# JiGuang283/Ray_Tracing-Rendering

Measured on AMD Instinct MI355X. Metric: Msamples/sec, Cornell Box 800x800 spp=400 MIS, higher is better.
Workload: dtype f64

## Files before the change

include/rtr_hip.h:

```cpp
#ifndef RTR_HIP_H
#define RTR_HIP_H

#include <stdint.h>
#include <stddef.h>

#ifdef __cplusplus
extern "C" {
#endif

#define RTR_ABI_VERSION 4

typedef enum rtr_status {
    RTR_OK = 0,
    RTR_ERR_INVALID = -1,
    RTR_ERR_UNSUPPORTED = -2,
    RTR_ERR_DEVICE = -3,
    RTR_ERR_NO_SCENE = -4,
    RTR_ERR_CANCELLED = -5,
    RTR_ERR_NOMEM = -6
} rtr_status;


typedef enum rtr_node_type {
    RTR_NODE_BVH = 0,
// ... 137 lines not shown
    int32_t max_depth;
    int32_t rr_start_depth;
    int32_t integrator;
    uint32_t seed;
    int32_t pipeline;
    int32_t tile_first;
    int32_t tile_stride;
    int32_t spp_chunks;
    int32_t flags;
} rtr_render_params;

#define RTR_FLAG_REFERENCE_ORDER 1
#define RTR_FLAG_WF_PERSISTENT 2
#define RTR_FLAG_SORTED_SHADING 4
#define RTR_FLAG_SPLIT_CASTS 8

typedef struct rtr_render_stats {
    uint64_t samples;
    uint64_t closest_segments;
    uint64_t shadow_segments;
    double device_ms;
    int32_t kernel_launches;
    int32_t pipeline;
    int32_t spp_chunks;
    int32_t cancelled;
    int32_t flags_in_effect;
    int32_t reserved;
} rtr_render_stats;

typedef struct rtr_context rtr_context;
// ... 198 lines not shown
```

ray_tracing-rendering_amd/_abi.py:

```python
import ctypes as C

import numpy as np

RTR_ABI_VERSION = 4

RTR_OK = 0
RTR_ERR_INVALID = -1
RTR_ERR_UNSUPPORTED = -2
RTR_ERR_DEVICE = -3
RTR_ERR_NO_SCENE = -4
RTR_ERR_CANCELLED = -5
RTR_ERR_NOMEM = -6

(NODE_BVH, NODE_LIST, NODE_TRANSLATE, NODE_ROTATE_Y, NODE_FLIP_FACE, NODE_MEDIUM, NODE_SPHERE,
 NODE_MOVING_SPHERE, NODE_XY_RECT, NODE_XZ_RECT, NODE_YZ_RECT) = range(11)
MAT_LAMBERTIAN, MAT_METAL, MAT_DIELECTRIC, MAT_DIFFUSE_LIGHT, MAT_PBR, MAT_ISOTROPIC = range(6)
TEX_SOLID, TEX_CHECKER, TEX_NOISE, TEX_IMAGE = range(4)
LIGHT_QUAD, LIGHT_POINT, LIGHT_SPOT, LIGHT_DIRECTIONAL, LIGHT_ENV_UNIFORM, LIGHT_ENV_MAP = 0, 1, 2, 3, 4, 5

INTEGRATOR_PATH, INTEGRATOR_RR, INTEGRATOR_PBR, INTEGRATOR_NEE, INTEGRATOR_MIS = 0, 1, 2, 3, 4
PIPELINE_AUTO, PIPELINE_MEGAKERNEL, PIPELINE_WAVEFRONT = 0, 1, 2
FLAG_REFERENCE_ORDER = 1
FLAG_WF_PERSISTENT = 2
FLAG_SORTED_SHADING = 4
FLAG_SPLIT_CASTS = 8
ACCUM_MOMENTS = 1

NODE_DTYPE = np.dtype([("type", "<i4"), ("a", "<i4"), ("b", "<i4"), ("reserved", "<i4"), ("f", "<f8", (10,))])
MATERIAL_DTYPE = np.dtype([("type", "<i4"), ("tex", "<i4", (4,)), ("reserved", "<i4", (3,)), ("f", "<f8", (4,))])
TEXTURE_DTYPE = np.dtype([("type", "<i4"), ("a", "<i4"), ("b", "<i4"), ("reserved", "<i4"), ("f", "<f8", (4,))])
PERLIN_DTYPE = np.dtype([("ranvec", "<f8", (256, 3)), ("perm_x", "<i4", (256,)), ("perm_y", "<i4", (256,)),
                         ("perm_z", "<i4", (256,))])
IMAGE_DTYPE = np.dtype([("width", "<i4"), ("height", "<i4"), ("offset", "<u8")])
LIGHT_DTYPE = np.dtype([("type", "<i4"), ("reserved", "<i4"), ("f", "<f8", (16,))])
CAMERA_DTYPE = np.dtype([("origin", "<f8", (3,)), ("lower_left_corner", "<f8", (3,)), ("horizontal", "<f8", (3,)),
                         ("vertical", "<f8", (3,)), ("u", "<f8", (3,)), ("v", "<f8", (3,)), ("w", "<f8", (3,)),
                         ("lens_radius", "<f8"), ("time0", "<f8"), ("time1", "<f8")])
assert NODE_DTYPE.itemsize == 96 and MATERIAL_DTYPE.itemsize == 64 and TEXTURE_DTYPE.itemsize == 48
assert PERLIN_DTYPE.itemsize == 9216 and IMAGE_DTYPE.itemsize == 16 and LIGHT_DTYPE.itemsize == 136
assert CAMERA_DTYPE.itemsize == 192
# ... 131 lines not shown
```

ray_tracing-rendering_amd/csrc/rt_kernels.h:

```cpp
#pragma once

#include "rt_render.h"

#ifndef RTR_MEGA_WAVES
#define RTR_MEGA_WAVES 4
#endif
#ifndef RTR_PROGRAM_WAVES
#define RTR_PROGRAM_WAVES 3
#endif

constexpr int mega_waves(int integ, int trav, int ms) {
    if (ms == RT_MS_LEAN) return RTR_MEGA_WAVES;
    if (rt_is_program(trav)) return RTR_PROGRAM_WAVES;
    if (trav == RT_TRAV_MEDIA || trav == RT_TRAV_EXACT) return 2;
    if (ms == RT_MS_QUADLIT) return 3;
    if (integ == RTR_INTEGRATOR_RR || integ == RTR_INTEGRATOR_PATH) return 3;
    return 2;
}

#define RT_PARK_WORDS 19
struct Park {
    double* base;
    RT_DEV V3 get3(int k) const { return mk(base[k * RTR_BLOCK], base[(k + 1) * RTR_BLOCK], base[(k + 2) * RTR_BLOCK]); }
    RT_DEV void set3(int k, V3 v) const {
// ... 521 lines not shown
    if (ACC == 2) P.q_part[(size_t)cell * RTR_BLOCK + threadIdx.x] = q;
    unsigned long long a = wave_sum(n_samples), b = wave_sum(cnt.closest), c = wave_sum(cnt.shadow);
    if ((threadIdx.x & 63) == 0) {
        atomicAdd(&P.stats[0], a);
        atomicAdd(&P.stats[1], b);
        atomicAdd(&P.stats[2], c);
    }
    const int interrupted = __syncthreads_or(active && s < s_end);
    if (threadIdx.x == 0) {
        P.done[cell] = !interrupted;
        if (interrupted) atomicAdd(&P.stats[7], 1ull);
    }
}


struct LiOut {
    double L[3];
    uint32_t rng_exit;
    int32_t n_closest, n_shadow, pad;
};
template <int INTEG, int TRAV>
__global__ void __launch_bounds__(RTR_BLOCK) k_li(const DScene sc, const RenderK P, const int32_t* __restrict__ ijs,
                                                   const rtr_li_ray* __restrict__ rays, LiOut* __restrict__ out, long long n) {
    extern __shared__ int lds_stack[];
    const Stack st{lds_stack + threadIdx.x};
    const long long k = (long long)blockIdx.x * RTR_BLOCK + threadIdx.x;
    if (k >= n) return;
    uint32_t rng;
    V3 ro, rd;
    Real tm;
// ... 145 lines not shown
    const bool cast = !rtr_ray_bad(r, media != 0);
    if (__any(cast && !(r.t_min >= 0x1p-100))) sc.shared_div = 0;
    if (cast) {
        blocked = cast_shadow<TRAV>(sc, ld3(r.origin), ld3(r.direction), r.t_max, rng, st, r.time, r.t_min);
    }
    occluded[k] = blocked ? 1 : 0;
    if (rng_out) rng_out[k] = rng;
}

#ifdef RTR_TU_CAPI
__global__ void __launch_bounds__(RTR_BLOCK) k_resolve(const ResolveK R) {
    const RenderK& P = R.r;
    int i, j;
    bool active;
    tile_pixel(P, blockIdx.x, threadIdx.x, i, j, active);
    for (int c = 0; c < P.chunks; ++c)
        if (!P.done[blockIdx.x * P.chunks + c]) return;
    const bool packed = R.row_stride < 0;
    if (packed && threadIdx.x == 0) R.tile_done[blockIdx.x] = 1;
    if (!active) return;
    const double* in = P.partial + (size_t)blockIdx.x * P.chunks * 3 * RTR_BLOCK + threadIdx.x;
    double r = 0, g = 0, b = 0;
    for (int c = 0; c < P.chunks; ++c) {
        if (c == 0) {
            r = in[0], g = in[RTR_BLOCK], b = in[2 * RTR_BLOCK];
        } else {
            r += in[0], g += in[RTR_BLOCK], b += in[2 * RTR_BLOCK];
        }
        in += 3 * RTR_BLOCK;
    }
    const double scale = 1.0 / P.spp;
    double* o = packed ? R.out + ((long long)blockIdx.x * RTR_BLOCK + threadIdx.x) * 3
// ... 615 lines not shown
```

ray_tracing-rendering_amd/csrc/rt_launch.h:

```cpp
#pragma once

#include "rt_render.h"

#include <atomic>
#include <string>
#include <utility>

struct LaunchedKernel {
    int trav = -1;
    int ms = -1;
    int sorted = 0;
    int phases = 0;
};

struct MegaVariant {
    int integ, trav, ms;
    bool sorted, pair;
};

struct MegaLaunch {
    MegaVariant variant;
    int accum;
    size_t lds;
    int stack_words;
    hipStream_t stream;
    const DScene* dsc;
    RenderK P;
    bool dry;
    int* blocks_per_cu;
};
int rtr_mega_launch_mis(const MegaLaunch& L, std::string& err);
int rtr_mega_launch_rr_path(const MegaLaunch& L, std::string& err);
int rtr_mega_launch_pbr_nee(const MegaLaunch& L, std::string& err);

void rtr_launch_resolve(const ResolveK& R, hipStream_t stream);

template <typename K>
int kernel_lds(K kernel, size_t dynamic_bytes, size_t static_bytes, std::string& err) {
    if (dynamic_bytes + static_bytes > 160 * 1024) {
        err = "this traversal of the scene needs a deeper stack than 160 KiB of LDS holds";
        return RTR_ERR_UNSUPPORTED;
    }
    if (dynamic_bytes <= 64 * 1024) return RTR_OK;
    const hipError_t e = hipFuncSetAttribute(reinterpret_cast<const void*>(kernel), hipFuncAttributeMaxDynamicSharedMemorySize,
// ... 32 lines not shown
```

ray_tracing-rendering_amd/csrc/rt_render.h:

```cpp
#pragma once

#include "rt_device.h"

struct RenderK {
    int W, H;
    int x0, y0, x1, y1;
    int spp, max_depth, rr_start;
    uint32_t seed;
    int tiles_x, tiles_y;
    const int* tile_ids;
    int n_tiles;
    int chunks;
    int n_big, big_spp, small_spp;
    int integrator;
    double* partial;
    unsigned long long* stats;
    const uint32_t* cancel;
    uint32_t render_id;
    int* done;
    const int* tile_s0;
    const double* acc_in;
    const int* tile_s1;
    const int* active;
    const int* n_active;
// ... 11 lines not shown
    const int tile = P.tile_ids[slot];
    const int tile_y = (P.tiles_y - 1) - tile / P.tiles_x;
    const int tile_x = tile % P.tiles_x;
    i = tile_x * 16 + (tid & 15);
    j = tile_y * 16 + (tid >> 4);
    active = i >= P.x0 && i < P.x1 && j >= P.y0 && j < P.y1;
}

RT_DEV void camera_sample(const DScene& sc, const RenderK& P, int i, int j, int s, uint32_t& rng, V3& ro, V3& rd, Real& tm) {
    rng = rtr_sample_seed_inline(P.seed, P.W, i, j, s);
    const Real u = (i + rng_next(rng)) / (P.W - 1);
    const Real v = (j + rng_next(rng)) / (P.H - 1);
    camera_get_ray(sc.camera, u, v, rng, ro, rd, tm);
}

RT_DEV void chunk_range(const RenderK& P, int c, int& s0, int& s1) {
    if (P.small_spp == 0) {
        s0 = (int)((long long)c * P.spp / P.chunks);
        s1 = (int)((long long)(c + 1) * P.spp / P.chunks);
    } else if (c < P.n_big) {
        s0 = c * P.big_spp, s1 = s0 + P.big_spp;
    } else {
        s0 = P.n_big * P.big_spp + (c - P.n_big) * P.small_spp, s1 = s0 + P.small_spp;
    }
    s0 = s0 < P.spp ? s0 : P.spp;
    s1 = s1 < P.spp ? s1 : P.spp;
    if (c == P.chunks - 1) s1 = P.spp;
}
RT_DEV void mega_work(const RenderK& P, int b, int& tile_slot, int& c) {
    if (P.small_spp == 0) {
        tile_slot = b / P.chunks, c = b % P.chunks;
    } else if (b < P.n_tiles * P.n_big) {
        tile_slot = b / P.n_big, c = b % P.n_big;
    } else {
        const int n_small = P.chunks - P.n_big, q = b - P.n_tiles * P.n_big;
        tile_slot = q / n_small, c = P.n_big + q % n_small;
    }
}

RT_DEV unsigned long long wave_sum(unsigned long long v) {
#pragma unroll
    for (int off = 32; off > 0; off >>= 1) v += __shfl_down(v, off, 64);
    return v;
}

struct ResolveK {
    RenderK r;
    double* out;
    long long row_stride;
    unsigned char* tile_done;
};

struct AccumResolveK {
    RenderK r;
    const double* sum;
    const int* count;
    double* out;
    unsigned char* rgb8;
};
```

ray_tracing-rendering_amd/csrc/rtr_capi.hip:

```cpp
#define RTR_TU_CAPI
#include "rt_lower.h"
#include "rt_kernels.h"
#include "rt_launch.h"
#include "rt_machine.h"
#include "rt_debug.h"

#include <atomic>
#include <cstdio>
#include <cstring>
#include <functional>
#include <map>
#include <mutex>
#include <string>
#include <vector>

namespace {

thread_local std::string g_create_error;

struct DevBuf {
    void* p = nullptr;
    size_t cap = 0;
};
struct SceneBufs {
// ... 372 lines not shown
int params_check(rtr_context* c, const rtr_render_params* p) {
    if (!p) return fail(c, RTR_ERR_INVALID, "null params");
    if (p->image_width < 2 || p->image_height < 2) return fail(c, RTR_ERR_INVALID, "image smaller than 2x2");
    if (((int64_t)p->image_width + 15) / 16 * (((int64_t)p->image_height + 15) / 16) > ((int64_t)1 << 26))
        return fail(c, RTR_ERR_INVALID, "image larger than 2^26 tiles");
    if (p->x0 < 0 || p->y0 < 0 || p->x1 > p->image_width || p->y1 > p->image_height || p->x0 >= p->x1 ||
        p->y0 >= p->y1)
        return fail(c, RTR_ERR_INVALID, "region outside the image or empty");
    if (p->spp < 1 || p->max_depth < 1 || p->rr_start_depth < 0)
        return fail(c, RTR_ERR_INVALID, "spp/max_depth/rr_start_depth out of range");
    if (p->integrator < RTR_INTEGRATOR_PATH || p->integrator > RTR_INTEGRATOR_MIS)
        return fail(c, RTR_ERR_UNSUPPORTED, "integrator id not supported (0 path, 1 RR, 2 PBR, 3 NEE, 4 MIS)");
    if (p->tile_stride > 1 && (p->tile_first < 0 || p->tile_first >= p->tile_stride))
        return fail(c, RTR_ERR_INVALID, "tile_first must be in [0, tile_stride)");
    if (p->spp_chunks < 0 || p->spp_chunks > p->spp) return fail(c, RTR_ERR_INVALID, "spp_chunks must be in [0, spp]");
    if (p->flags & ~(RTR_FLAG_REFERENCE_ORDER | RTR_FLAG_WF_PERSISTENT | RTR_FLAG_SORTED_SHADING | RTR_FLAG_SPLIT_CASTS)) return fail(c, RTR_ERR_INVALID, "unknown flag bits");
    if (p->pipeline < RTR_PIPELINE_AUTO || p->pipeline > RTR_PIPELINE_WAVEFRONT)
        return fail(c, RTR_ERR_INVALID, "unknown pipeline");
    return RTR_OK;
}

std::vector<int> owned_tiles(const rtr_render_params& p, int& tiles_x, int& tiles_y) {
    tiles_x = (p.image_width + 15) / 16;
    tiles_y = (p.image_height + 15) / 16;
    const int stride = p.tile_stride > 1 ? p.tile_stride : 1;
    const int first = p.tile_stride > 1 ? p.tile_first : 0;
    std::vector<int> out;
    for (int t = first; t < tiles_x * tiles_y; t += stride) {
        int ty = (tiles_y - 1) - t / tiles_x, tx = t % tiles_x;
        int xs = tx * 16, ys = ty * 16;
        if (xs + 16 <= p.x0 || xs >= p.x1 || ys + 16 <= p.y0 || ys >= p.y1) continue;
// ... 40 lines not shown
    if (v.trav == RT_TRAV_PROGRAM && (f.guarded_program || n1)) v.trav = RT_TRAV_PROGRAM_EXT;
    if (n1) {
        if (v.trav == RT_TRAV_EXACT) v.trav = RT_TRAV_MEDIA;
        return v;
    }
    const int t = v.trav;
    const bool lean = f.lean_materials && (t == RT_TRAV_FLAT || t == RT_TRAV_FAST || t == RT_TRAV_TOP || t == RT_TRAV_EXACT);
    const bool quadlit = f.quad_lights_only && !f.needs_uv && integ == RTR_INTEGRATOR_MIS && t != RT_TRAV_MEDIA && t != RT_TRAV_EXACT;
    v.ms = lean ? RT_MS_LEAN : (quadlit ? RT_MS_QUADLIT : RT_MS_FULL);
    v.sorted = (flags & RTR_FLAG_SORTED_SHADING) && f.n_materials <= 65535 && mega_sortable(integ, t, v.ms);
    const bool pairable = mega_pairable(integ, t) && !v.sorted && f.pair_cast;
    v.pair = pairable && !(flags & RTR_FLAG_SPLIT_CASTS);
    if (flags_in_effect && v.sorted) *flags_in_effect |= RTR_FLAG_SORTED_SHADING;
    if (flags_in_effect && pairable && !v.pair) *flags_in_effect |= RTR_FLAG_SPLIT_CASTS;
    return v;
}

int launch_mega(rtr_context* c, const RenderK& P, int integrator, int trav_in, bool dry, int* blocks_per_cu, int flags,
                int* flags_in_effect = nullptr, LaunchedKernel* launched = nullptr) {
    MegaLaunch L{};
    const MegaVariant& v = L.variant = mega_variant(c->facts, integrator, trav_in, flags, flags_in_effect);
    L.stack_words = (int)(stack_bytes(c->facts, c->info, v.trav) / (RTR_BLOCK * sizeof(int)));
    L.dsc = static_cast<const DScene*>(c->sb.dscene.p);
    const int park = v.sorted ? SK_WORDS : park_words(integrator, trav_in == RT_TRAV_EXACT ? RT_TRAV_EXACT : v.trav);
    L.lds = stack_bytes(c->facts, c->info, v.trav) + (size_t)park * RTR_BLOCK * sizeof(double);
    L.accum = P.tile_s0 == nullptr ? 0 : (P.q_in ? 2 : 1);
    L.stream = c->stream;
    L.P = P;
    L.dry = dry;
    L.blocks_per_cu = blocks_per_cu;
    int rc;
    switch (integrator) {
    case RTR_INTEGRATOR_MIS: rc = rtr_mega_launch_mis(L, c->err); break;
    case RTR_INTEGRATOR_RR:
    case RTR_INTEGRATOR_PATH: rc = rtr_mega_launch_rr_path(L, c->err); break;
    default: rc = rtr_mega_launch_pbr_nee(L, c->err); break;
    }
    if (rc == RTR_OK && !dry && launched) launched->trav = v.trav, launched->ms = v.ms, launched->sorted = v.sorted;
    return rc;
}

int auto_chunks(int pipeline, double resident_slots, int n_tiles, int spp) {
    int chunks = 1;
    if (pipeline == RTR_PIPELINE_WAVEFRONT) {
        while ((long long)n_tiles * chunks < 8192 && chunks * 2 * 8 <= spp && chunks < 64) chunks *= 2;
// ... 109 lines not shown
        return RTR_OK;
    }
    HIPCHK(c, hipEventSynchronize(c->ev1));
    float ms = 0;
    HIPCHK(c, hipEventElapsedTime(&ms, c->ev0, c->ev1));
    unsigned long long h[RT_STATS_WORDS] = {0};
    HIPCHK(c, hipMemcpy(h, c->b_stats.p, sizeof h, hipMemcpyDeviceToHost));
    if (getenv("RTR_REGION_PROFILE")) {
        static const char* names[RG_N] = {"other / loop", "closest: instance setup", "closest: rect runs", "closest: sphere runs",
                                          "closest: generic scan", "closest: tree inner nodes", "closest: tree leaves",
                                          "closest: hit record (fast_finish)", "shadow: instance setup", "shadow: rect runs",
                                          "shadow: sphere runs", "shadow: generic scan", "shadow: tree inner nodes",
                                          "shadow: tree leaves", "media steps", "mat_prepare", "shade_a (emission, light sample)",
                                          "shade_b (BSDF sample, roulette)", "miss", "end of sample + regeneration",
                                          "shade_rr / shade_path", "park path state", "sorted shading: barrier waits",
                                          "sorted shading: tickets + exchange", "pair cast: instance setup",
                                          "pair cast: rect runs", "pair cast: sphere runs", "sample end: cancel poll",
                                          "sample end: begin_sample (camera ray)", "sample end: settle into the pixel sum",
                                          "cast counters", "random_in_unit_sphere rejection loop"};
        double total = 0;
        for (int k = 0; k < RG_N; ++k) total += (double)h[RT_PROF_BASE + k];
        std::fprintf(stderr, "[region profile] %.4g wave cycles in all, %llu samples\n", total, h[0]);
        for (int k = 0; k < RG_N; ++k)
            if (h[RT_PROF_BASE + RT_PROF_REGIONS + k])
                std::fprintf(stderr, "[region profile] %-36s %6.2f %%  %12llu visits  %8.1f cycles/visit\n", names[k],
                             100.0 * (double)h[RT_PROF_BASE + k] / total, h[RT_PROF_BASE + RT_PROF_REGIONS + k],
                             (double)h[RT_PROF_BASE + k] / (double)h[RT_PROF_BASE + RT_PROF_REGIONS + k]);
    }
#ifdef RTR_PHASE_CLOCKS
    std::fprintf(stderr, "[phase clocks] closest %.3e  shade %.3e  shadow %.3e  other %.3e (wave cycles)\n", (double)h[3],
                 (double)h[4], (double)h[5], (double)h[6]);
// ... 219 lines not shown
    if (pipeline == RTR_PIPELINE_AUTO) pipeline = RTR_PIPELINE_MEGAKERNEL;
    const int trav = pick_trav(c->facts, c->info, p->flags);
    if (pipeline == RTR_PIPELINE_WAVEFRONT && (!c->facts.machine_ok || (trav != RT_TRAV_FLAT && trav != RT_TRAV_FAST && trav != RT_TRAV_PROGRAM)))
        return fail(c, RTR_ERR_UNSUPPORTED, "the wavefront pipeline runs the compiled traversals only: this graph (or "
                                            "RTR_FLAG_REFERENCE_ORDER) needs the reference-order walk of the megakernel");
    if (pipeline == RTR_PIPELINE_WAVEFRONT && (p->flags & RTR_FLAG_WF_PERSISTENT) && c->facts.guarded_program)
        return fail(c, RTR_ERR_UNSUPPORTED, "RTR_FLAG_WF_PERSISTENT: the traversal machine does not run step programs with "
                                            "guarded primitives (hollow spheres under bvh_nodes) or media under transforms; "
                                            "the lockstep stages do");
    int chunks = p->spp_chunks, guided[3] = {0, 0, 0};
    if (chunks == 0 && (rc = choose_chunks(c, P, p->integrator, pipeline, trav, p->spp, p->flags, &chunks, guided))) return rc;
    P.n_big = guided[0], P.big_spp = guided[1], P.small_spp = guided[2];
    P.chunks = chunks;

    const size_t partial_bytes = (size_t)P.n_tiles * chunks * 3 * RTR_BLOCK * sizeof(double);
    const size_t done_bytes = (size_t)P.n_tiles * chunks * sizeof(int);
    const bool same_tiles = acc || tiles == c->last_tiles;
    if ((c->stats_pending || c->in_flight) && (!same_tiles || partial_bytes > c->b_partial.cap || done_bytes > c->b_done.cap ||
                                               pipeline == RTR_PIPELINE_WAVEFRONT)) {
        if ((rc = finish_stats(c))) return rc;
    }
    if (!same_tiles) {
        c->last_tiles.clear();
        if ((rc = upload(c, c->b_tiles, tiles.data(), tiles.size() * sizeof(int)))) return rc;
        c->last_tiles = tiles;
    }
    if ((rc = ensure(c, c->b_partial, partial_bytes))) return rc;
    if ((rc = ensure(c, c->b_done, done_bytes))) return rc;
    P.tile_ids = static_cast<const int*>(acc ? acc->d_tiles.p : c->b_tiles.p);
    if (acc) {
        P.tile_s0 = static_cast<const int*>(acc->d_count.p);
        P.acc_in = static_cast<const double*>(acc->d_sum.p);
        P.tile_s1 = static_cast<const int*>(acc->d_s1.p);
        P.active = static_cast<const int*>(acc->d_active.p);
        P.n_active = static_cast<const int*>(acc->d_nactive.p);
        if (acc->moments) {
            P.q_in = static_cast<const double*>(acc->d_q.p);
            P.q_part = static_cast<double*>(acc->d_qpart.p);
        }
    }
    P.stats = static_cast<unsigned long long*>(c->b_stats.p);
    P.cancel = static_cast<const uint32_t*>(c->b_cancel.p);
    P.partial = static_cast<double*>(c->b_partial.p);
    P.done = static_cast<int*>(c->b_done.p);
    if (pipeline == RTR_PIPELINE_MEGAKERNEL && (rc = launch_mega(c, P, p->integrator, trav, true, nullptr, p->flags))) return rc;

    const uint32_t id = c->render_seq.fetch_add(1) + 1;
    P.render_id = id;
    c->stats_pending = false;
    c->in_flight = true;
    c->stats = rtr_render_stats{};
    c->stats.spp_chunks = chunks;
    c->last_kernel = rtr_debug_kernel{-1, -1, -1, -1, 0, 0, 0, 0, 0, 0, 0};
    LaunchedKernel launched{};
    c->pending_id = id;
    HIPCHK(c, hipMemsetAsync(c->b_stats.p, 0, RT_STATS_WORDS * sizeof(unsigned long long), c->stream));
    if (c->camera_dirty) {
        hipLaunchKernelGGL(k_camera_store, dim3(1), dim3(64), 0, c->stream, static_cast<DScene*>(c->sb.dscene.p), c->ds.camera);
        HIPCHK(c, hipGetLastError());
        c->camera_dirty = false;
// ... 27 lines not shown
            K.n_tiles = P.n_tiles;
            K.count = static_cast<const int*>(acc->d_count.p);
            K.err = static_cast<const double*>(acc->d_err.p);
            K.tile_s1 = static_cast<int*>(acc->d_s1.p);
            K.active = static_cast<int*>(acc->d_active.p);
            K.n_active = static_cast<int*>(acc->d_nactive.p);
            if (K.mode == 2) {
                hipLaunchKernelGGL(k_accum_errors, dim3((unsigned)P.n_tiles), dim3(RTR_BLOCK), 0, c->stream, accum_view(acc),
                                   static_cast<const double*>(acc->d_q.p), static_cast<double*>(acc->d_err.p));
                ++launches;
            }
            hipLaunchKernelGGL(k_accum_plan, dim3(1), dim3(1024), 0, c->stream, K);
            ++launches;
            HIPCHK(c, hipGetLastError());
        }
        if ((rc = launch_mega(c, P, p->integrator, trav, false, nullptr, p->flags, &c->stats.flags_in_effect, &launched))) return rc;
        c->last_kernel = rtr_debug_kernel{pipeline, p->integrator, launched.trav, launched.ms, launched.sorted, 0, 0, 0, 0, 0, 0,
                                          acc ? (acc->moments ? 2 : 1) : 0};
        if (acc) {
            hipLaunchKernelGGL(k_accum_commit, dim3((unsigned)P.n_tiles), dim3(RTR_BLOCK), 0, c->stream, P,
                               static_cast<double*>(acc->d_sum.p), static_cast<double*>(acc->moments ? acc->d_q.p : nullptr),
                               static_cast<int*>(acc->d_count.p));
        } else {
            ResolveK R{P, d_rgb, (long long)row_stride, tile_done};
            rtr_launch_resolve(R, c->stream);
        }
        HIPCHK(c, hipGetLastError());
        c->stats.kernel_launches = launches;
    }
    HIPCHK(c, hipEventRecord(c->ev1, c->stream));
    c->stats.pipeline = pipeline;
    c->stats_pending = true;
    if (blocking || c->stats.cancelled) {
        HIPCHK(c, hipStreamSynchronize(c->stream));
        if ((rc = finish_stats(c))) return rc;
        if (c->stats.cancelled) return fail(c, RTR_ERR_CANCELLED, "render cancelled");
    }
    return RTR_OK;
}
// ... 1193 lines not shown
```

ray_tracing-rendering_amd/csrc/rtr_mega.hip:

```cpp
#include "rt_kernels.h"
#include "rt_launch.h"

#ifndef RTR_MEGA_GROUP
#error "compile with -DRTR_MEGA_GROUP=0|1|2"
#endif

namespace {

int mega_fail(std::string& err, int code, const std::string& m) {
    err = m;
    return code;
}

template <typename K>
int launch_one(K kernel, const MegaLaunch& L, std::string& err) {
    hipFuncAttributes fa{};
    hipError_t e = hipFuncGetAttributes(&fa, reinterpret_cast<const void*>(kernel));
    if (e == hipSuccess)
        if (int rc = kernel_lds(kernel, L.lds, fa.sharedSizeBytes, err)) return rc;
    if (e == hipSuccess && L.dry && L.blocks_per_cu)
        e = hipOccupancyMaxActiveBlocksPerMultiprocessor(L.blocks_per_cu, kernel, RTR_BLOCK, L.lds);
    if (e == hipSuccess && !L.dry) {
        hipLaunchKernelGGL(kernel, dim3((unsigned)(L.P.n_tiles * L.P.chunks)), dim3(RTR_BLOCK), L.lds, L.stream, L.dsc, L.P,
                           L.stack_words);
        e = hipGetLastError();
    }
    if (e != hipSuccess) return mega_fail(err, RTR_ERR_DEVICE, std::string("megakernel launch: ") + hipGetErrorString(e));
    return RTR_OK;
}

template <int I, int T, int M, bool S = false, bool PR = false>
struct Row {
    static bool is(const MegaVariant& v) { return v.integ == I && v.trav == T && v.ms == M && v.sorted == S && v.pair == PR; }
    static int launch(const MegaLaunch& L, std::string& err) {
        return L.accum == 2 ? launch_one(k_mega<I, T, M, S, 2, PR>, L, err)
               : L.accum    ? launch_one(k_mega<I, T, M, S, 1, PR>, L, err)
                            : launch_one(k_mega<I, T, M, S, 0, PR>, L, err);
    }
};
template <typename... Rows>
int launch_from(const MegaLaunch& L, std::string& err) {
    int rc = RTR_OK;
    if (((Rows::is(L.variant) && (rc = Rows::launch(L, err), true)) || ...)) return rc;
    const MegaVariant& v = L.variant;
    return mega_fail(err, RTR_ERR_UNSUPPORTED,
                     "no megakernel instantiation for integrator " + std::to_string(v.integ) + ", traversal " + std::to_string(v.trav) +
                         ", material set " + std::to_string(v.ms) + (v.sorted ? ", sorted" : "") + (v.pair ? ", pair cast" : ""));
}

// ... 65 lines not shown
```

ray_tracing-rendering_amd/native.py:

```python
import ctypes as C
import os
import weakref

import numpy as np

from . import _abi as A
from .scene import Scene

_HERE = os.path.dirname(os.path.abspath(__file__))
_LIB = None

_STATUS = {A.RTR_ERR_INVALID: "RTR_ERR_INVALID", A.RTR_ERR_UNSUPPORTED: "RTR_ERR_UNSUPPORTED",
           A.RTR_ERR_DEVICE: "RTR_ERR_DEVICE", A.RTR_ERR_NO_SCENE: "RTR_ERR_NO_SCENE",
           A.RTR_ERR_CANCELLED: "RTR_ERR_CANCELLED", A.RTR_ERR_NOMEM: "RTR_ERR_NOMEM"}

EXPORTS = ("rtr_abi_version", "rtr_device_count", "rtr_create", "rtr_destroy", "rtr_set_stream",
           "rtr_upload_scene", "rtr_render_device", "rtr_render_host", "rtr_render_tiles_host", "rtr_plan_chunks", "rtr_li_samples", "rtr_li_rays",
           "rtr_synchronize", "rtr_cancel", "rtr_get_stats", "rtr_last_error", "rtr_sample_seed", "rtr_validate_scene",
           "rtr_accum_create", "rtr_accum_render", "rtr_accum_resolve", "rtr_accum_tiles", "rtr_accum_destroy",
           "rtr_accum_create_ex", "rtr_accum_render_tiles", "rtr_accum_moments", "rtr_accum_errors", "rtr_accum_refine",
           "rtr_denoise_defaults", "rtr_accum_features", "rtr_accum_denoise", "rtr_denoise_host",
           "rtr_query_closest", "rtr_query_occluded", "rtr_query_closest_device", "rtr_query_occluded_device",
           "rtr_set_camera", "rtr_get_camera", "rtr_accum_reset", "rtr_temporal_defaults", "rtr_history_create",
           "rtr_history_clear", "rtr_history_destroy", "rtr_history_planes", "rtr_accum_denoise_temporal",
           "rtr_display_defaults", "rtr_display_srgb_thresholds", "rtr_display_histogram", "rtr_display_host",
           "rtr_display_device", "rtr_accum_resolve_device", "rtr_accum_features_device", "rtr_accum_denoise_device",
           "rtr_accum_denoise_temporal_device")
TEST_EXPORTS = ("rtr_test_hits", "rtr_test_materials", "rtr_test_lights", "rtr_test_li", "rtr_test_reference_order",
                "rtr_test_stream8", "rtr_test_sincos_exhaustive", "rtr_test_shared_division", "rtr_test_issue_rates", "rtr_test_last_kernel",
                "rtr_test_temporal_planes", "rtr_test_scene_plan", "rtr_test_flat_hits", "rtr_test_pair_frames",
                "rtr_test_pair_frame_host", "rtr_test_pair_cast")
_TEST_LIB = None


class SceneInfoC(C.Structure):
    _fields_ = [("stack_words", C.c_int32), ("has_media", C.c_int32), ("needs_uv", C.c_int32),
                ("graph_depth", C.c_int32), ("fast_ok", C.c_int32), ("fast_instances", C.c_int32),
                ("fast_refs", C.c_int32), ("fast_stack_words", C.c_int32), ("compiled_subtrees", C.c_int32),
                ("program_steps", C.c_int32), ("inverted_boxes", C.c_int32), ("top_trees", C.c_int32)]


class KernelRecordC(C.Structure):
    _fields_ = [(name, C.c_int32) for name in ("pipeline", "integrator", "trav", "ms", "sorted", "shade_phases", "lean",
                                               "quadlit", "sort", "media", "machine", "accum")]


# ... 2 lines not shown
        "fast_ok", "has_media", "flat_scene", "flat_guarded", "lean_materials", "quad_lights_only", "uv_order_dependent",
        "machine_ok", "guarded_program", "top_tree", "needs_uv", "n_material_types", "shared_div", "pair_cast", "n_steps",
        "n_visits", "n_refs", "fast_stack_words", "walk_stack_words", "n_tie_refs", "n_guard_refs", "pick_trav", "mega_trav",
        "mega_ms", "mega_sorted", "mega_pair", "n_finish")]


FINISH_DTYPE = np.dtype([("kind", "<i4"), ("material", "<i4"), ("levels", "<i4"), ("flip", "<i4"), ("op", "<f8", (2, 3)),
                         ("g", "<f8", (4,))])


PAIR_FRAME_DTYPE = np.dtype([("ao", "<f8", (3,)), ("ad", "<f8", (3,)), ("bo", "<f8", (3,)), ("bd", "<f8", (3,)),
                             ("fo", "<f8", (3,)), ("fd", "<f8", (3,)), ("same_frame", "<i4"), ("pad", "<i4")])
PAIR_DTYPE = np.dtype([("ao", "<f8", (3,)), ("ad", "<f8", (3,)), ("a_tmax", "<f8"), ("bo", "<f8", (3,)), ("bd", "<f8", (3,)),
                       ("b_tmax", "<f8"), ("a_t", "<f8"), ("s_a_t", "<f8"), ("a_ref", "<i4"), ("a_inst", "<i4"),
                       ("b_hit", "<i4"), ("s_a_ref", "<i4"), ("s_a_inst", "<i4"), ("s_b_hit", "<i4")])
FRAME_SHAPES = ("none", "T", "R", "TR", "RT", "other")


class RtrError(RuntimeError):
    def __init__(self, code, message):
        super().__init__("%s (%d): %s" % (_STATUS.get(code, "rtr_status"), code, message))
        self.code = code
        self.message = message


def library_path():
    return os.environ.get("RTR_HIP_LIBRARY") or os.path.join(_HERE, "librtr_hip.so")


def lib():
# ... 91 lines not shown
    T.rtr_test_li.argtypes = [vp, C.POINTER(A.RenderParamsC), vp, C.c_int64]
    T.rtr_test_reference_order.argtypes = [vp, C.c_int]
    T.rtr_test_stream8.argtypes = [vp, C.c_int64, C.c_int]
    T.rtr_test_sincos_exhaustive.argtypes = [vp, C.POINTER(C.c_uint64), C.POINTER(C.c_uint64)]
    T.rtr_test_issue_rates.argtypes = [vp, C.POINTER(C.c_double), C.c_int]
    T.rtr_test_shared_division.argtypes = [vp, C.POINTER(C.c_uint64), C.POINTER(C.c_uint64)]
    T.rtr_test_last_kernel.argtypes = [vp, C.POINTER(KernelRecordC), C.c_size_t]
    T.rtr_test_temporal_planes.argtypes = [vp] + [C.c_int32] * 6 + [C.POINTER(A.CameraC), C.POINTER(A.CameraC), C.c_int,
                                                                    C.POINTER(A.TemporalParamsC)] + [vp] * 8
    T.rtr_test_scene_plan.argtypes = [C.POINTER(A.SceneDescC), C.c_int32, C.c_int32, C.POINTER(ScenePlanC), vp, C.c_int64,
                                      vp, C.c_int64]
    T.rtr_test_flat_hits.argtypes = [vp, vp, C.c_int64, C.c_int, C.POINTER(C.c_int32)]
    T.rtr_test_pair_frames.argtypes = [C.POINTER(A.SceneDescC), vp, C.c_int64, C.POINTER(C.c_int32)]
    T.rtr_test_pair_frame_host.argtypes = [C.c_int32, vp, vp, C.c_int64]
    T.rtr_test_pair_cast.argtypes = [vp, vp, C.c_int64]
    _TEST_LIB = T
    return T


def validate_scene(scene):
    L = lib()
    d = scene.desc()
    info = SceneInfoC()
    msg = C.create_string_buffer(256)
    rc = L.rtr_validate_scene(C.byref(d), C.byref(info), msg, len(msg))
    if rc != 0:
        raise RtrError(rc, msg.value.decode())
    return {"stack_words": info.stack_words, "has_media": bool(info.has_media), "needs_uv": bool(info.needs_uv),
            "graph_depth": info.graph_depth, "fast_ok": bool(info.fast_ok), "fast_instances": info.fast_instances,
            "fast_refs": info.fast_refs, "fast_stack_words": info.fast_stack_words,
# ... 26 lines not shown
    if rc != 0:
        raise RtrError(rc, "scene rejected")
    shapes = np.zeros(n.value, dtype=np.int32)
    T.rtr_test_pair_frames(C.byref(d), shapes.ctypes.data, len(shapes), C.byref(n))
    return [FRAME_SHAPES[k] for k in shapes]


def pair_frame_host(shape, ops, ao, ad, bo, bd):
    recs = np.zeros(len(ao), dtype=PAIR_FRAME_DTYPE)
    recs["ao"], recs["ad"], recs["bo"], recs["bd"] = ao, ad, bo, bd
    ops = np.ascontiguousarray(ops, dtype=np.float64).reshape(6)
    rc = test_lib().rtr_test_pair_frame_host(FRAME_SHAPES.index(shape), ops.ctypes.data, recs.ctypes.data, len(recs))
    if rc != 0:
        raise RtrError(rc, "rtr_test_pair_frame_host")
    return recs


def denoise_defaults(**overrides):
    p = A.DenoiseParamsC()
    lib().rtr_denoise_defaults(C.byref(p))
    for k, v in overrides.items():
        if k not in ("iterations", "feature_spp", "sigma_l", "sigma_n", "sigma_a", "sigma_z"):
            raise TypeError("no denoise parameter %r" % k)
        setattr(p, k, v)
    return p


def temporal_defaults(**overrides):
    p = A.TemporalParamsC()
    lib().rtr_temporal_defaults(C.byref(p))
# ... 540 lines not shown
```

Before: 5414.

## Add persistent megakernel with atomic work queue for pixel-sample jobs

Result: faster. 5734, median of 6 (+5.9%).

```diff
diff --git a/include/rtr_hip.h b/include/rtr_hip.h
--- a/include/rtr_hip.h
+++ b/include/rtr_hip.h
@@ -175,6 +175,7 @@
 #define RTR_FLAG_WF_PERSISTENT 2
 #define RTR_FLAG_SORTED_SHADING 4
 #define RTR_FLAG_SPLIT_CASTS 8
+#define RTR_FLAG_STATIC_GRID 16
 
 typedef struct rtr_render_stats {
     uint64_t samples;
diff --git a/ray_tracing-rendering_amd/_abi.py b/ray_tracing-rendering_amd/_abi.py
--- a/ray_tracing-rendering_amd/_abi.py
+++ b/ray_tracing-rendering_amd/_abi.py
@@ -24,6 +24,7 @@
 FLAG_WF_PERSISTENT = 2
 FLAG_SORTED_SHADING = 4
 FLAG_SPLIT_CASTS = 8
+FLAG_STATIC_GRID = 16
 ACCUM_MOMENTS = 1
 
 NODE_DTYPE = np.dtype([("type", "<i4"), ("a", "<i4"), ("b", "<i4"), ("reserved", "<i4"), ("f", "<f8", (10,))])
diff --git a/ray_tracing-rendering_amd/csrc/rt_kernels.h b/ray_tracing-rendering_amd/csrc/rt_kernels.h
--- a/ray_tracing-rendering_amd/csrc/rt_kernels.h
+++ b/ray_tracing-rendering_amd/csrc/rt_kernels.h
@@ -559,6 +559,246 @@
 }
 
 
+struct QueueWave {
+    int block;
+    int next;
+    unsigned long long samples;
+};
+RT_DEV bool queue_take(const RenderK& P, uint32_t* __restrict__ q_counter, const int n_blocks, QueueWave& qw, bool need,
+                       const Park& pk, int* my_cell, int& s) {
+    bool got = false;
+    unsigned long long m = __ballot(need);
+    while (m) {
+        if (qw.block >= 0 && qw.next == RT_QUEUE_JOBS) {
+            const int first = __builtin_ctzll(m);
+            uint32_t b = 0;
+            if ((int)__lane_id() == first) b = atomicAdd(q_counter, 1u);
+            b = (uint32_t)__builtin_amdgcn_readlane((int)b, first);
+            qw.block = b < (uint32_t)n_blocks ? (int)b : -1;
+            qw.next = 0;
+        }
+        if (qw.block < 0) {
+            if (need) *my_cell = -1;
+            break;
+        }
+        const QueueBlock qb = queue_block(P, qw.block);
+        const int tile = P.tile_ids[qb.slot];
+        const int tile_y = (P.tiles_y - 1) - tile / P.tiles_x;
+        const int tile_x = tile % P.tiles_x;
+        const int cell = qb.slot * P.chunks + qb.chunk;
+        const int k = qw.next + (int)__builtin_amdgcn_mbcnt_hi((uint32_t)(m >> 32), __builtin_amdgcn_mbcnt_lo((uint32_t)m, 0u));
+        bool now = false;
+        if (need && k < RT_QUEUE_JOBS) {
+            const int i = tile_x * 16 + (k & 15), j = tile_y * 16 + qb.quarter * 4 + (k >> 4);
+            if (i >= P.x0 && i < P.x1 && j >= P.y0 && j < P.y1 && qb.s0 < qb.s1) {
+                uint32_t lo, hi;
+                queue_pack(i, j, qb.s1, lo, hi);
+                pk.set2(PK_PIXEL, lo, hi);
+                *my_cell = cell;
+                s = qb.s0;
+                got = now = true, need = false;
+            } else {
+                atomicAdd(&P.done[cell], 1);
+            }
+        }
+        qw.samples += (unsigned long long)__builtin_popcountll(__ballot(now)) * (unsigned long long)(qb.s1 - qb.s0);
+        const int taken = qw.next + (int)__builtin_popcountll(m);
+        qw.next = taken < RT_QUEUE_JOBS ? taken : RT_QUEUE_JOBS;
+        m = __ballot(need);
+    }
+    return got;
+}
+
+template <int INTEG, int TRAV, int MS>
+__global__ void __launch_bounds__(RTR_BLOCK, mega_waves(INTEG, TRAV, MS))
+    k_mega_queue(const DScene* __restrict__ scp, const RenderK P, const int stack_words, uint32_t* __restrict__ q_counter,
+                 const int n_blocks) {
+    static_assert(mega_pairable(INTEG, TRAV), "no pair-cast variant of this kernel");
+    extern __shared__ int lds_stack[];
+    const DScene& sc = *scp;
+    const Stack st{lds_stack + threadIdx.x};
+    const Park pk{reinterpret_cast<double*>(lds_stack + stack_words * RTR_BLOCK) + threadIdx.x};
+    int* const my_cell = lds_stack + threadIdx.x;
+#ifdef RTR_REGION_PROFILE
+    if (threadIdx.x < 4 * 2 * RT_PROF_REGIONS + 8) rt_prof_lds[threadIdx.x] = 0;
+    if (threadIdx.x + 256 < 4 * 2 * RT_PROF_REGIONS + 8) rt_prof_lds[threadIdx.x + 256] = 0;
+    __syncthreads();
+    if ((threadIdx.x & 63) == 0) rt_prof_lds[4 * 2 * RT_PROF_REGIONS + (threadIdx.x >> 6) * 2] = __builtin_readcyclecounter();
+#endif
+    PathCounters cnt;
+    cnt.closest = 0, cnt.shadow = 0;
+    PathState ps;
+    uint32_t rng = 1;
+    int s = 0;
+    QueueWave qw{0, RT_QUEUE_JOBS, 0ull};
+    pk.set3(PK_ACC, mk(0.0, 0.0, 0.0));
+    pk.set2(PK_NCAST, 0u, 0u);
+    pk.set3(PK_L, mk(0.0, 0.0, 0.0));
+    *my_cell = -1;
+    bool done = !queue_take(P, q_counter, n_blocks, qw, true, pk, my_cell, s);
+    if (!done) {
+        uint32_t lo, hi;
+        int i, j, s_end;
+        pk.get2(PK_PIXEL, lo, hi);
+        queue_unpack(lo, hi, i, j, s_end);
+        camera_sample(sc, P, i, j, s, rng, ps.ro, ps.rd, ps.tm);
+        ps.depth = 0, ps.specular_bounce = false;
+        pk.set3(PK_THR, mk(1.0, 1.0, 1.0));
+        pk.set(PK_PDF, 0.0);
+    }
+    uint32_t it = 0;
+    bool pending = false;
+    bool settle = false;
+    V3 so = mk(0.0, 0.0, 0.0);
+    PhaseClocks clk;
+    while (!done || settle) {
+        RTR_CLK(other);
+        RT_REGION(RG_OTHER);
+        const bool cast_a = !done;
+        Real a_tmax = RT_INF, b_tmax = 0.0;
+        int a_ref, a_inst, b_ref;
+        V3 swi = mk(1.0, 1.0, 1.0);
+        RT_REGION(RG_COUNT);
+        {
+            uint32_t n_closest, n_shadow;
+            pk.get2(PK_NCAST, n_closest, n_shadow);
+            pk.set2(PK_NCAST, n_closest + (cast_a ? 1u : 0u), n_shadow + (pending ? 1u : 0u));
+        }
+        RT_REGION(RG_OTHER);
+        if (!cast_a) {
+            ps.ro = mk(0.0, 0.0, 0.0), ps.rd = mk(1.0, 1.0, 1.0), ps.tm = 0.0;
+            a_tmax = 0.0;
+        }
+        if (pending) {
+            swi = pk.get3(PK_SWI);
+            b_tmax = pk.get(PK_STMAX);
+        } else {
+            so = mk(0.0, 0.0, 0.0);
+        }
+        trace_pair(sc, ps.ro, ps.rd, ps.tm, a_tmax, a_ref, a_inst, so, swi, b_tmax, b_ref, st);
+        RTR_CLK(closest);
+        RT_REGION(RG_POLL);
+        const uint32_t cancel_word = cancel_poll_issue(P, it++);
+        RT_REGION(RG_SETTLE);
+        const bool lit = pending && b_ref < 0;
+        if (lit || settle) {
+            V3 L = pk.get3(PK_L);
+            if (lit) L = add(L, pk.get3(PK_CONTRIB));
+            if (settle) {
+                pk.set3(PK_ACC, add(pk.get3(PK_ACC), L));
+                L = mk(0.0, 0.0, 0.0);
+                settle = false;
+            }
+            pk.set3(PK_L, L);
+        }
+        pending = false;
+        RTR_CLK(shadow);
+        bool begin = false;
+        if (cast_a) {
+            bool ended;
+            if (a_ref < 0) {
+                RT_REGION(RG_MISS);
+                pk.set3(PK_L, add(pk.get3(PK_L), miss_radiance<INTEG, MS>(sc, pk.get3(PK_THR), ps.ro, ps.rd, ps.depth,
+                                                                      ps.specular_bounce, pk.get(PK_PDF))));
+                ended = true;
+            } else {
+                Hit rec;
+                rec.u = 0, rec.v = 0;
+                if (MS == RT_MS_FULL && sc.needs_uv)
+                    fast_finish<true, true>(sc, ps.ro, ps.rd, ps.tm, a_tmax, a_ref, a_inst, rec);
+                else
+                    fast_finish<false, true>(sc, ps.ro, ps.rd, ps.tm, a_tmax, a_ref, a_inst, rec);
+                ps.thr = pk.get3(PK_THR);
+                ps.L = mk(0.0, 0.0, 0.0);
+                ps.prev_bsdf_pdf = pk.get(PK_PDF);
+                const V3 wo = neg(unit(ps.rd));
+                ParkedReq rq{false, pk};
+                const MatCtx mc = mat_prepare<MS>(sc, rec);
+                shade_a_mis<MS, INTEG>(sc, ps, rec, mc, wo, rng, rq);
+                pending = rq.valid;
+                const bool go = shade_b_mis<MS, INTEG>(sc, ps, rec, mc, wo, rng, P.rr_start);
+                RT_REGION(RG_PARK);
+                ps.ro = rec.p;
+                so = rec.p;
+                pk.set3(PK_THR, ps.thr);
+                if (ps.L.x != 0.0 || ps.L.y != 0.0 || ps.L.z != 0.0) pk.set3(PK_L, add(pk.get3(PK_L), ps.L));
+                pk.set(PK_PDF, ps.prev_bsdf_pdf);
+                ended = !go || ++ps.depth >= P.max_depth;
+            }
+            RTR_CLK(shade);
+            RT_REGION(RG_REGEN);
+            if (ended) {
+                settle = true;
+                ++s;
+                begin = true;
+            }
+        }
+        const bool job_end = !cast_a && *my_cell >= 0;
+        if (__ballot(job_end)) {
+            RT_REGION(RG_EXCHANGE);
+            if (job_end) {
+                uint32_t lo, hi;
+                pk.get2(PK_PIXEL, lo, hi);
+                const V3 acc = pk.get3(PK_ACC);
+                const int cell = *my_cell;
+                double* out = P.partial + (size_t)cell * 3 * RTR_BLOCK + ((lo >> 12) & 0xf0u) + (lo & 0xfu);
+                out[0] = acc.x;
+                out[RTR_BLOCK] = acc.y;
+                out[2 * RTR_BLOCK] = acc.z;
+                atomicAdd(&P.done[cell], 1);
+                pk.set3(PK_ACC, mk(0.0, 0.0, 0.0));
+            }
+            if (queue_take(P, q_counter, n_blocks, qw, job_end, pk, my_cell, s)) done = false, begin = true;
+        }
+        if (begin) {
+            uint32_t lo, hi;
+            int i, j, s_end;
+            pk.get2(PK_PIXEL, lo, hi);
+            queue_unpack(lo, hi, i, j, s_end);
+            done = s >= s_end;
+            if (!done) {
+                RT_REGION(RG_BEGIN);
+                camera_sample(sc, P, i, j, s, rng, ps.ro, ps.rd, ps.tm);
+                ps.depth = 0, ps.specular_bounce = false;
+                pk.set3(PK_THR, mk(1.0, 1.0, 1.0));
+                pk.set(PK_PDF, 0.0);
+            }
+        }
+        RT_REGION(RG_POLL);
+        if (__any(cancel_poll_take(P, cancel_word))) {
+            const unsigned long long here = __ballot(1);
+            if ((int)__lane_id() == __builtin_ctzll(here)) atomicAdd(&P.stats[7], 1ull);
+            int left = 0;
+            if (*my_cell >= 0) {
+                uint32_t lo, hi;
+                pk.get2(PK_PIXEL, lo, hi);
+                left = (int)hi - s;
+            }
+            for (unsigned long long m = __ballot(left > 0); m; m &= m - 1)
+                qw.samples -= (unsigned long long)__builtin_amdgcn_readlane(left, __builtin_ctzll(m));
+            *my_cell = -1;
+            done = true;
+        }
+    }
+    pk.get2(PK_NCAST, cnt.closest, cnt.shadow);
+    clk.flush(P);
+#ifdef RTR_REGION_PROFILE
+    RT_REGION(RG_OTHER);
+    __syncthreads();
+    if (threadIdx.x < 2 * RT_PROF_REGIONS) {
+        unsigned long long v = 0;
+        for (int w = 0; w < 4; ++w) v += rt_prof_lds[w * 2 * RT_PROF_REGIONS + threadIdx.x];
+        if (v) atomicAdd(&P.stats[RT_PROF_BASE + threadIdx.x], v);
+    }
+#endif
+    unsigned long long b = wave_sum(cnt.closest), c = wave_sum(cnt.shadow);
+    if ((threadIdx.x & 63) == 0) {
+        atomicAdd(&P.stats[0], qw.samples);
+        atomicAdd(&P.stats[1], b);
+        atomicAdd(&P.stats[2], c);
+    }
+}
+
 struct LiOut {
     double L[3];
     uint32_t rng_exit;
@@ -734,8 +974,10 @@
     int i, j;
     bool active;
     tile_pixel(P, blockIdx.x, threadIdx.x, i, j, active);
-    for (int c = 0; c < P.chunks; ++c)
-        if (!P.done[blockIdx.x * P.chunks + c]) return;
+    for (int c = 0; c < P.chunks; ++c) {
+        const int d = P.done[blockIdx.x * P.chunks + c];
+        if (R.done_full ? d != R.done_full : !d) return;
+    }
     const bool packed = R.row_stride < 0;
     if (packed && threadIdx.x == 0) R.tile_done[blockIdx.x] = 1;
     if (!active) return;
diff --git a/ray_tracing-rendering_amd/csrc/rt_launch.h b/ray_tracing-rendering_amd/csrc/rt_launch.h
--- a/ray_tracing-rendering_amd/csrc/rt_launch.h
+++ b/ray_tracing-rendering_amd/csrc/rt_launch.h
@@ -28,6 +28,8 @@
     RenderK P;
     bool dry;
     int* blocks_per_cu;
+    bool queue;
+    int n_cus, grid_cap;
 };
 int rtr_mega_launch_mis(const MegaLaunch& L, std::string& err);
 int rtr_mega_launch_rr_path(const MegaLaunch& L, std::string& err);
diff --git a/ray_tracing-rendering_amd/csrc/rt_render.h b/ray_tracing-rendering_amd/csrc/rt_render.h
--- a/ray_tracing-rendering_amd/csrc/rt_render.h
+++ b/ray_tracing-rendering_amd/csrc/rt_render.h
@@ -49,7 +49,7 @@
     camera_get_ray(sc.camera, u, v, rng, ro, rd, tm);
 }
 
-RT_DEV void chunk_range(const RenderK& P, int c, int& s0, int& s1) {
+RT_HD void chunk_range(const RenderK& P, int c, int& s0, int& s1) {
     if (P.small_spp == 0) {
         s0 = (int)((long long)c * P.spp / P.chunks);
         s1 = (int)((long long)(c + 1) * P.spp / P.chunks);
@@ -62,7 +62,7 @@
     s1 = s1 < P.spp ? s1 : P.spp;
     if (c == P.chunks - 1) s1 = P.spp;
 }
-RT_DEV void mega_work(const RenderK& P, int b, int& tile_slot, int& c) {
+RT_HD void mega_work(const RenderK& P, int b, int& tile_slot, int& c) {
     if (P.small_spp == 0) {
         tile_slot = b / P.chunks, c = b % P.chunks;
     } else if (b < P.n_tiles * P.n_big) {
@@ -71,6 +71,25 @@
         const int n_small = P.chunks - P.n_big, q = b - P.n_tiles * P.n_big;
         tile_slot = q / n_small, c = P.n_big + q % n_small;
     }
+}
+
+#define RT_QUEUE_JOBS 64
+struct QueueBlock {
+    int slot, quarter, chunk;
+    int s0, s1;
+};
+RT_HD QueueBlock queue_block(const RenderK& P, int b) {
+    QueueBlock q;
+    mega_work(P, b >> 2, q.slot, q.chunk);
+    q.quarter = b & 3;
+    chunk_range(P, q.chunk, q.s0, q.s1);
+    return q;
+}
+RT_HD void queue_pack(int i, int j, int s_end, uint32_t& lo, uint32_t& hi) {
+    lo = (uint32_t)i | ((uint32_t)j << 16), hi = (uint32_t)s_end;
+}
+RT_HD void queue_unpack(uint32_t lo, uint32_t hi, int& i, int& j, int& s_end) {
+    i = (int)(lo & 0xffffu), j = (int)(lo >> 16), s_end = (int)hi;
 }
 
 RT_DEV unsigned long long wave_sum(unsigned long long v) {
@@ -84,6 +103,7 @@
     double* out;
     long long row_stride;
     unsigned char* tile_done;
+    int done_full;
 };
 
 struct AccumResolveK {
diff --git a/ray_tracing-rendering_amd/csrc/rtr_capi.hip b/ray_tracing-rendering_amd/csrc/rtr_capi.hip
--- a/ray_tracing-rendering_amd/csrc/rtr_capi.hip
+++ b/ray_tracing-rendering_amd/csrc/rtr_capi.hip
@@ -410,7 +410,7 @@
     if (p->tile_stride > 1 && (p->tile_first < 0 || p->tile_first >= p->tile_stride))
         return fail(c, RTR_ERR_INVALID, "tile_first must be in [0, tile_stride)");
     if (p->spp_chunks < 0 || p->spp_chunks > p->spp) return fail(c, RTR_ERR_INVALID, "spp_chunks must be in [0, spp]");
-    if (p->flags & ~(RTR_FLAG_REFERENCE_ORDER | RTR_FLAG_WF_PERSISTENT | RTR_FLAG_SORTED_SHADING | RTR_FLAG_SPLIT_CASTS)) return fail(c, RTR_ERR_INVALID, "unknown flag bits");
+    if (p->flags & ~(RTR_FLAG_REFERENCE_ORDER | RTR_FLAG_WF_PERSISTENT | RTR_FLAG_SORTED_SHADING | RTR_FLAG_SPLIT_CASTS | RTR_FLAG_STATIC_GRID)) return fail(c, RTR_ERR_INVALID, "unknown flag bits");
     if (p->pipeline < RTR_PIPELINE_AUTO || p->pipeline > RTR_PIPELINE_WAVEFRONT)
         return fail(c, RTR_ERR_INVALID, "unknown pipeline");
     return RTR_OK;
@@ -481,6 +481,11 @@
     if (flags_in_effect && v.sorted) *flags_in_effect |= RTR_FLAG_SORTED_SHADING;
     if (flags_in_effect && pairable && !v.pair) *flags_in_effect |= RTR_FLAG_SPLIT_CASTS;
     return v;
+}
+
+bool mega_queue(const MegaVariant& v, const RenderK& P, int flags) {
+    return v.pair && P.tile_s0 == nullptr && !(flags & RTR_FLAG_STATIC_GRID) && P.W <= 65535 && P.H <= 65535 &&
+           (long long)P.n_tiles * P.chunks * 4 < (1ll << 31);
 }
 
 int launch_mega(rtr_context* c, const RenderK& P, int integrator, int trav_in, bool dry, int* blocks_per_cu, int flags,
@@ -496,6 +501,10 @@
     L.P = P;
     L.dry = dry;
     L.blocks_per_cu = blocks_per_cu;
+    L.queue = mega_queue(v, P, flags);
+    L.n_cus = c->n_cus;
+    if (const char* g = getenv("RTR_QUEUE_WORKGROUPS")) L.grid_cap = std::atoi(g);
+    if (flags_in_effect && v.pair && L.accum == 0 && (flags & RTR_FLAG_STATIC_GRID)) *flags_in_effect |= RTR_FLAG_STATIC_GRID;
     int rc;
     switch (integrator) {
     case RTR_INTEGRATOR_MIS: rc = rtr_mega_launch_mis(L, c->err); break;
@@ -635,7 +644,7 @@
                                           "shadow: tree leaves", "media steps", "mat_prepare", "shade_a (emission, light sample)",
                                           "shade_b (BSDF sample, roulette)", "miss", "end of sample + regeneration",
                                           "shade_rr / shade_path", "park path state", "sorted shading: barrier waits",
-                                          "sorted shading: tickets + exchange", "pair cast: instance setup",
+                                          "sorted shading: tickets + exchange / queue: job switch", "pair cast: instance setup",
                                           "pair cast: rect runs", "pair cast: sphere runs", "sample end: cancel poll",
                                           "sample end: begin_sample (camera ray)", "sample end: settle into the pixel sum",
                                           "cast counters", "random_in_unit_sphere rejection loop"};
@@ -885,7 +894,7 @@
     P.chunks = chunks;
 
     const size_t partial_bytes = (size_t)P.n_tiles * chunks * 3 * RTR_BLOCK * sizeof(double);
-    const size_t done_bytes = (size_t)P.n_tiles * chunks * sizeof(int);
+    const size_t done_bytes = ((size_t)P.n_tiles * chunks + 1) * sizeof(int);
     const bool same_tiles = acc || tiles == c->last_tiles;
     if ((c->stats_pending || c->in_flight) && (!same_tiles || partial_bytes > c->b_partial.cap || done_bytes > c->b_done.cap ||
                                                pipeline == RTR_PIPELINE_WAVEFRONT)) {
@@ -915,6 +924,7 @@
     P.partial = static_cast<double*>(c->b_partial.p);
     P.done = static_cast<int*>(c->b_done.p);
     if (pipeline == RTR_PIPELINE_MEGAKERNEL && (rc = launch_mega(c, P, p->integrator, trav, true, nullptr, p->flags))) return rc;
+    const bool queue = pipeline == RTR_PIPELINE_MEGAKERNEL && mega_queue(mega_variant(c->facts, p->integrator, trav, p->flags, nullptr), P, p->flags);
 
     const uint32_t id = c->render_seq.fetch_add(1) + 1;
     P.render_id = id;
@@ -972,6 +982,8 @@
             ++launches;
             HIPCHK(c, hipGetLastError());
         }
+        if (queue)
+            HIPCHK(c, hipMemsetAsync(c->b_done.p, 0, done_bytes, c->stream));
         if ((rc = launch_mega(c, P, p->integrator, trav, false, nullptr, p->flags, &c->stats.flags_in_effect, &launched))) return rc;
         c->last_kernel = rtr_debug_kernel{pipeline, p->integrator, launched.trav, launched.ms, launched.sorted, 0, 0, 0, 0, 0, 0,
                                           acc ? (acc->moments ? 2 : 1) : 0};
@@ -980,7 +992,7 @@
                                static_cast<double*>(acc->d_sum.p), static_cast<double*>(acc->moments ? acc->d_q.p : nullptr),
                                static_cast<int*>(acc->d_count.p));
         } else {
-            ResolveK R{P, d_rgb, (long long)row_stride, tile_done};
+            ResolveK R{P, d_rgb, (long long)row_stride, tile_done, queue ? RTR_BLOCK : 0};
             rtr_launch_resolve(R, c->stream);
         }
         HIPCHK(c, hipGetLastError());
diff --git a/ray_tracing-rendering_amd/csrc/rtr_mega.hip b/ray_tracing-rendering_amd/csrc/rtr_mega.hip
--- a/ray_tracing-rendering_amd/csrc/rtr_mega.hip
+++ b/ray_tracing-rendering_amd/csrc/rtr_mega.hip
@@ -29,10 +29,34 @@
     return RTR_OK;
 }
 
+template <typename K>
+int launch_queue(K kernel, const MegaLaunch& L, std::string& err) {
+    hipFuncAttributes fa{};
+    hipError_t e = hipFuncGetAttributes(&fa, reinterpret_cast<const void*>(kernel));
+    if (e == hipSuccess)
+        if (int rc = kernel_lds(kernel, L.lds, fa.sharedSizeBytes, err)) return rc;
+    int per_cu = 0;
+    if (e == hipSuccess) e = hipOccupancyMaxActiveBlocksPerMultiprocessor(&per_cu, kernel, RTR_BLOCK, L.lds);
+    if (e == hipSuccess && L.dry && L.blocks_per_cu) *L.blocks_per_cu = per_cu;
+    if (e == hipSuccess && !L.dry) {
+        const long long cells = (long long)L.P.n_tiles * L.P.chunks;
+        long long grid = (long long)(per_cu > 0 ? per_cu : 1) * (L.n_cus > 0 ? L.n_cus : 1);
+        if (grid > cells) grid = cells;
+        if (L.grid_cap > 0 && grid > L.grid_cap) grid = L.grid_cap;
+        hipLaunchKernelGGL(kernel, dim3((unsigned)grid), dim3(RTR_BLOCK), L.lds, L.stream, L.dsc, L.P, L.stack_words,
+                           reinterpret_cast<uint32_t*>(L.P.done + cells), (int)(cells * 4));
+        e = hipGetLastError();
+    }
+    if (e != hipSuccess) return mega_fail(err, RTR_ERR_DEVICE, std::string("megakernel launch: ") + hipGetErrorString(e));
+    return RTR_OK;
+}
+
 template <int I, int T, int M, bool S = false, bool PR = false>
 struct Row {
     static bool is(const MegaVariant& v) { return v.integ == I && v.trav == T && v.ms == M && v.sorted == S && v.pair == PR; }
     static int launch(const MegaLaunch& L, std::string& err) {
+        if constexpr (PR)
+            if (L.queue) return launch_queue(k_mega_queue<I, T, M>, L, err);
         return L.accum == 2 ? launch_one(k_mega<I, T, M, S, 2, PR>, L, err)
                : L.accum    ? launch_one(k_mega<I, T, M, S, 1, PR>, L, err)
                             : launch_one(k_mega<I, T, M, S, 0, PR>, L, err);
diff --git a/ray_tracing-rendering_amd/native.py b/ray_tracing-rendering_amd/native.py
--- a/ray_tracing-rendering_amd/native.py
+++ b/ray_tracing-rendering_amd/native.py
@@ -29,7 +29,7 @@
 TEST_EXPORTS = ("rtr_test_hits", "rtr_test_materials", "rtr_test_lights", "rtr_test_li", "rtr_test_reference_order",
                 "rtr_test_stream8", "rtr_test_sincos_exhaustive", "rtr_test_shared_division", "rtr_test_issue_rates", "rtr_test_last_kernel",
                 "rtr_test_temporal_planes", "rtr_test_scene_plan", "rtr_test_flat_hits", "rtr_test_pair_frames",
-                "rtr_test_pair_frame_host", "rtr_test_pair_cast")
+                "rtr_test_pair_frame_host", "rtr_test_pair_cast", "rtr_test_queue_blocks_host", "rtr_test_queue_pack_host")
 _TEST_LIB = None
 
 
@@ -62,6 +62,7 @@
 PAIR_DTYPE = np.dtype([("ao", "<f8", (3,)), ("ad", "<f8", (3,)), ("a_tmax", "<f8"), ("bo", "<f8", (3,)), ("bd", "<f8", (3,)),
                        ("b_tmax", "<f8"), ("a_t", "<f8"), ("s_a_t", "<f8"), ("a_ref", "<i4"), ("a_inst", "<i4"),
                        ("b_hit", "<i4"), ("s_a_ref", "<i4"), ("s_a_inst", "<i4"), ("s_b_hit", "<i4")])
+QUEUE_BLOCK_DTYPE = np.dtype([(name, "<i4") for name in ("slot", "quarter", "chunk", "s0", "s1", "ref_s0", "ref_s1", "pad")])
 FRAME_SHAPES = ("none", "T", "R", "TR", "RT", "other")
 
 
@@ -183,6 +184,8 @@
     T.rtr_test_pair_frames.argtypes = [C.POINTER(A.SceneDescC), vp, C.c_int64, C.POINTER(C.c_int32)]
     T.rtr_test_pair_frame_host.argtypes = [C.c_int32, vp, vp, C.c_int64]
     T.rtr_test_pair_cast.argtypes = [vp, vp, C.c_int64]
+    T.rtr_test_queue_blocks_host.argtypes = [C.c_int32] * 6 + [vp, C.c_int64]
+    T.rtr_test_queue_pack_host.argtypes = [C.c_int32] * 3 + [C.POINTER(C.c_uint32), C.POINTER(C.c_uint32), vp]
     _TEST_LIB = T
     return T
 
@@ -239,6 +242,23 @@
     if rc != 0:
         raise RtrError(rc, "rtr_test_pair_frame_host")
     return recs
+
+
+def queue_blocks_host(n_tiles, spp, chunks, guided=(0, 0, 0)):
+    recs = np.zeros(n_tiles * chunks * 4, dtype=QUEUE_BLOCK_DTYPE)
+    rc = test_lib().rtr_test_queue_blocks_host(n_tiles, spp, chunks, *[int(g) for g in guided], recs.ctypes.data, len(recs))
+    if rc != 0:
+        raise RtrError(rc, "rtr_test_queue_blocks_host")
+    return recs
+
+
+def queue_pack_host(i, j, s_end):
+    lo, hi = C.c_uint32(0), C.c_uint32(0)
+    out = np.zeros(3, dtype=np.int32)
+    rc = test_lib().rtr_test_queue_pack_host(int(i), int(j), int(s_end), C.byref(lo), C.byref(hi), out.ctypes.data)
+    if rc != 0:
+        raise RtrError(rc, "rtr_test_queue_pack_host")
+    return (lo.value, hi.value), tuple(int(v) for v in out)
 
 
 def denoise_defaults(**overrides):
```
